# mfkiwl/msckf_stereo_c

Hardware: AMD Instinct MI355X
Metric: stereo frames/sec/node on EuRoC-shape input; ATE RMSE vs CPU ref (higher is better)
Workload: dtype f64

## Files before the change

### msckf_stereo_c_amd/csrc/hip/fe_kernels.hip

```cpp
#include <stdlib.h>
#include <mutex>
#include "fe_device.h"
#include "fe_mask.h"

__device__ __forceinline__ int reflect101(int i, int n) {
    if (n == 1) return 0;
    while (i < 0 || i >= n) { i = (i < 0) ? -i : 2 * (n - 1) - i; }
    return i;
}

#define P3_HALO 2
#define P3_OWN 12
#define P3_SEG_ROWS 8
struct Pyr3Job { const uint8_t *src; uint8_t *d1, *d2, *d3; int w0, h0; };

namespace {
typedef uint32_t __attribute__((aligned(1))) pd_u32u;
typedef uint16_t __attribute__((aligned(1))) pd_u16u;
typedef unsigned long long __attribute__((aligned(1))) pd_u64u;
typedef const __attribute__((address_space(1))) pd_u64u *pd_gld64;
typedef __attribute__((address_space(1))) pd_u32u *pd_gst32;
typedef __attribute__((address_space(1))) pd_u16u *pd_gst16;
typedef __attribute__((address_space(1))) uint8_t *pd_gst8;

// ... 209 lines not shown
    const int job = 4 * wi + (lane >> 4);
    const int seg = job / strips, strip = job - seg * strips;
    const int xs = DET_BORDER + DS_COLS * strip;
    const int ys = DET_BORDER + seg_rows * seg;
    const int y_end = min(ys + seg_rows, H - DET_BORDER);
    const bool job_on = xs < W - DET_BORDER && ys < y_end;
    if (!__any(job_on)) return;
    const int c0 = xs - 4 + 4 * r;
    const int cl = min(c0, W - 4);
    const uint8_t *img = S.curr0.lvl[0];
    typedef uint32_t __attribute__((aligned(1))) u32u;
    auto load = [&](int row) -> DetPix {
        const uint8_t *p = img + (size_t)min(max(row, 0), H - 1) * W + cl;
        DetPix v; v.lo = *(const u32u *)(p - 4); v.hi = *(const u32u *)p; return v;
    };
    int xin[4], cx[4];
    bool col_ok[4];
#pragma unroll
    for (int j = 0; j < 4; ++j) {
        const int x = c0 + 4 + j;
        cx[j] = x / cw; xin[j] = x - cx[j] * cw;
        col_ok[j] = job_on && r < DS_LANES && x < W - DET_BORDER;
    }
    const uint32_t *mrow = nullptr;
    int mpw = 0, msh = 0;
    if constexpr (MASKED) {
        mrow = masks[si].mask0; mpw = masks[si].pitch_w;
        if (mrow) mrow += min(c0 + 4, W - 1) >> 5;
        msh = (c0 + 4) & 31;
    }
    int Va[4] = {0, 0, 0, 0}, Vb[4] = {0, 0, 0, 0}, Vc[4] = {0, 0, 0, 0};
    int pr = ys - 4;
    DetPix e_mid = load(pr), e_dn = load(pr + 1), e_nx = load(pr + 2);
    uint32_t e_up = load(pr - 1).hi;
#pragma unroll 1
    for (int k = 0; k < 8; ++k) {
        const DetPix nx = load(pr + 3);
        int P[12];
        det_prod(e_up, e_mid, e_dn.hi, P);
        det_vadd(P, Va, Vb, Vc);
        e_up = e_mid.hi; e_mid = e_dn; e_dn = e_nx; e_nx = nx; ++pr;
    }
    uint32_t l_up = load(ys - 5).hi;
    DetPix l_mid = load(ys - 4), l_dn = load(ys - 3), l_nx = load(ys - 2);
    int cy = ys / ch, yin = ys - cy * ch;
    int bs[4] = {0, 0, 0, 0};
    unsigned long long bk[4] = {0ULL, 0ULL, 0ULL, 0ULL};
    const int n_rows = seg_rows;
#pragma unroll 1
    for (int k = 0; k < n_rows; ++k) {
        const int y = ys + k;
        const bool row_ok = y < y_end;
        const DetPix enx = load(pr + 3), lnx = load(y - 1);
        uint32_t nib = 15u;
        if constexpr (MASKED) { if (mrow) nib = (mrow[(size_t)min(y, H - 1) * mpw] >> msh) & 15u; }
        if (!MASKED || nib)
#pragma unroll
        for (int j = 0; j < 4; ++j) {
            if (!(col_ok[j] && row_ok)) continue;
            if (MASKED && !((nib >> j) & 1u)) continue;
            const int a = Va[j], b = Vb[j], d = Vc[j];
            const int X = (a + d) - max(det_floor, bs[j]);
            if (X <= 0) continue;
            const int df = a - d;
            if (abs(df) >= X || 2 * abs(b) >= X) continue;
            const double discd = (double)df * (double)df + 4.0 * ((double)b * (double)b);
            if (discd >= (double)X * (double)X) continue;
            const long long disc = (long long)df * df + 4LL * ((long long)b * b);
            const int score = (a + d) - (int)isqrt48((unsigned long long)disc, discd);
            bs[j] = score;
            bk[j] = det_key(gen, score, (unsigned int)(yin * cw + xin[j]));
        }
        {
            int Pe[12], Pl[12];
            det_prod(e_up, e_mid, e_dn.hi, Pe);
            det_prod(l_up, l_mid, l_dn.hi, Pl);
#pragma unroll
            for (int j = 0; j < 12; ++j) Pe[j] -= Pl[j];
            det_vadd(Pe, Va, Vb, Vc);
            e_up = e_mid.hi; e_mid = e_dn; e_dn = e_nx; e_nx = enx; ++pr;
            l_up = l_mid.hi; l_mid = l_dn; l_dn = l_nx; l_nx = lnx;
        }
        ++yin;
        const bool flush = job_on && row_ok && (yin == ch || y + 1 == y_end);
        if (cw < 4) {
            if (flush) {
#pragma unroll
                for (int j = 0; j < 4; ++j) {
                    if (bk[j]) atomicMax(&cell_keys[cy * det_cols + cx[j]], bk[j]);
                    bs[j] = 0; bk[j] = 0ULL;
                }
            }
        } else if (__any(flush)) {
            unsigned long long ka = 0ULL, kb = 0ULL;
#pragma unroll
            for (int j = 0; j < 4; ++j) {
                const unsigned long long v = flush ? bk[j] : 0ULL;
                if (cx[j] == cx[0]) ka = v > ka ? v : ka; else kb = v > kb ? v : kb;
            }
            const bool two = cx[3] != cx[0];
#pragma unroll 1
            for (int pass = 0; pass < 2; ++pass) {
                unsigned long long kk = pass ? kb : ka;
                const int id = flush ? (pass ? (two ? cx[3] : -1 - r) : cx[0]) : -1 - r;
                if (pass && !__any(flush && two)) break;
                {
                    const int o = det_dpp0<0x101>(id + 0x40000000) - 0x40000000; const unsigned long long v = det_dpp0_64<0x101>(kk);
                    if (o == id && v > kk) kk = v;
                }
                {
                    const int o = det_dpp0<0x102>(id + 0x40000000) - 0x40000000; const unsigned long long v = det_dpp0_64<0x102>(kk);
                    if (o == id && v > kk) kk = v;
                }
                {
                    const int o = det_dpp0<0x104>(id + 0x40000000) - 0x40000000; const unsigned long long v = det_dpp0_64<0x104>(kk);
                    if (o == id && v > kk) kk = v;
                }
                {
                    const int o = det_dpp0<0x108>(id + 0x40000000) - 0x40000000; const unsigned long long v = det_dpp0_64<0x108>(kk);
                    if (o == id && v > kk) kk = v;
                }
                const int left = det_dpp0<0x111>(id + 0x40000000) - 0x40000000;
                if (id >= 0 && left != id && kk) atomicMax(&cell_keys[cy * det_cols + id], kk);
            }
            if (flush) {
#pragma unroll
                for (int j = 0; j < 4; ++j) { bs[j] = 0; bk[j] = 0ULL; }
            }
        }
        if (yin == ch) { yin = 0; ++cy; }
    }
}

static void det_launch(const FeStreamDev *streams_dev, const FeMaskDev *masks_dev, int n_streams, int max_w, int max_h, unsigned int gen, hipStream_t st) {
    const int strips = (max_w - 2 * DET_BORDER + DS_COLS - 1) / DS_COLS, rows = max_h - 2 * DET_BORDER;
    if (strips <= 0 || rows <= 0) return;
    int seg_rows = 32;
    while (seg_rows < 128 && (long long)n_streams * strips * ((rows + seg_rows - 1) / seg_rows) / 4 > 32768) seg_rows *= 2;
    const int segs = (rows + seg_rows - 1) / seg_rows;
    const int waves = (strips * segs + 3) / 4;
    if (masks_dev) hipLaunchKernelGGL(k_detect_cells<true>, dim3(8 * ((n_streams + 7) / 8) * waves), dim3(64), 0, st, streams_dev, masks_dev, n_streams, strips, seg_rows, waves, gen);
    else hipLaunchKernelGGL(k_detect_cells<false>, dim3(8 * ((n_streams + 7) / 8) * waves), dim3(64), 0, st, streams_dev, masks_dev, n_streams, strips, seg_rows, waves, gen);
}
extern "C" void fe_launch_detect(const FeStreamDev *streams_dev, int n_streams, int max_w, int max_h, unsigned int gen, hipStream_t st) {
    det_launch(streams_dev, nullptr, n_streams, max_w, max_h, gen, st);
}
extern "C" void fe_launch_detect_masked(const FeStreamDev *streams_dev, const FeMaskDev *masks_dev, int n_streams, int max_w, int max_h, unsigned int gen, hipStream_t st) {
    if (!masks_dev) return;
    det_launch(streams_dev, masks_dev, n_streams, max_w, max_h, gen, st);
}

#include "fe_cam_models.h"

__device__ __forceinline__ void undistort_pt(const CamDev &cam, const double *R, float u, float v, float &xo, float &yo) {
    const double fx = cam.K[0], fy = cam.K[1], cx = cam.K[2], cy = cam.K[3];
    double x = ((double)u - cx) / fx, y = ((double)v - cy) / fy;
    if (cam.model == MSKF_MODEL_EQUIDISTANT) {
        const double *k = cam.D;
        double theta_d = sqrt(x * x + y * y);
        const double half_pi = 1.5707963267948966;
        theta_d = theta_d > half_pi ? half_pi : (theta_d < -half_pi ? -half_pi : theta_d);
        double scale = 0.0;
        if (theta_d > 1e-8) {
            double theta = theta_d;
            for (int j = 0; j < 10; ++j) {
                const double t2 = theta * theta, t4 = t2 * t2, t6 = t4 * t2, t8 = t6 * t2;
                const double k0t2 = k[0] * t2, k1t4 = k[1] * t4, k2t6 = k[2] * t6, k3t8 = k[3] * t8;
                const double fix = (theta * (1 + k0t2 + k1t4 + k2t6 + k3t8) - theta_d) /
                                   (1 + 3 * k0t2 + 5 * k1t4 + 7 * k2t6 + 9 * k3t8);
                theta = theta - fix;
                if (fabs(fix) < 1e-8) break;
            }
            scale = det_tan(theta) / theta_d;
        }
        x = x * scale; y = y * scale;
    } else {
        const double k1 = cam.D[0], k2 = cam.D[1], p1 = cam.D[2], p2 = cam.D[3];
        const double x0 = x, y0 = y;
        for (int j = 0; j < 5; ++j) {
            const double r2 = x * x + y * y;
            const double icdist = 1.0 / (1.0 + (k2 * r2 + k1) * r2);
            const double deltaX = 2.0 * p1 * x * y + p2 * (r2 + 2.0 * x * x);
            const double deltaY = p1 * (r2 + 2.0 * y * y) + 2.0 * p2 * x * y;
            x = (x0 - deltaX) * icdist;
            y = (y0 - deltaY) * icdist;
        }
    }
    if (R) {
        const double X = R[0] * x + R[1] * y + R[2];
        const double Y = R[3] * x + R[4] * y + R[5];
        const double Wd = R[6] * x + R[7] * y + R[8];
        x = X / Wd; y = Y / Wd;
    } else {
        x = x / 1.0; y = y / 1.0;
    }
    xo = (float)(x * 1.0 + 0.0);
    yo = (float)(y * 1.0 + 0.0);
}

__device__ __forceinline__ void distort_pt(const CamDev &cam, float xf, float yf, float &uo, float &vo) {
    const double fx = cam.K[0], fy = cam.K[1], cx = cam.K[2], cy = cam.K[3];
    const double x = (double)xf, y = (double)yf;
    double xd, yd;
    if (cam.model == MSKF_MODEL_EQUIDISTANT) {
        const double *k = cam.D;
        const double r = sqrt(x * x + y * y);
        const double theta = det_atan(r);
        const double t2 = theta * theta, t4 = t2 * t2, t6 = t4 * t2, t8 = t4 * t4;
        const double theta_d = theta * (1 + k[0] * t2 + k[1] * t4 + k[2] * t6 + k[3] * t8);
        const double scale = (r > 1e-8) ? theta_d / r : 1.0;
        xd = x * scale; yd = y * scale;
    } else {
        const double k1 = cam.D[0], k2 = cam.D[1], p1 = cam.D[2], p2 = cam.D[3];
        const double r2 = x * x + y * y, r4 = r2 * r2;
        const double a1 = 2.0 * x * y, a2 = r2 + 2.0 * x * x, a3 = r2 + 2.0 * y * y;
        const double cdist = 1.0 + k1 * r2 + k2 * r4;
        xd = x * cdist + p1 * a1 + p2 * a2;
        yd = y * cdist + p1 * a3 + p2 * a1;
    }
    uo = (float)(xd * fx + cx);
    vo = (float)(yd * fy + cy);
}

__device__ __forceinline__ bool undistort_pt_ext(const CamDev &cam, int model, const double *coef, const double *R, float u, float v, float &xo, float &yo) {
    if (model < FCM_RADTAN8) { undistort_pt(cam, R, u, v, xo, yo); return true; }
    return fcm_undistort_px(cam.K, model, coef, R, u, v, xo, yo);
}
__device__ __forceinline__ bool distort_pt_ext(const CamDev &cam, int model, const double *coef, float xf, float yf, float &uo, float &vo) {
    if (model < FCM_RADTAN8) { distort_pt(cam, xf, yf, uo, vo); return true; }
    return fcm_distort_px(cam.K, model, coef, xf, yf, uo, vo);
}

#include "fe_lk.h"

template <bool EXT>
__device__ __forceinline__ void track4_body(const FeStreamDev *streams, const FeCamExtDev *exts, int n_streams, int groups_per_stream,
                                            uint32_t (*s_T)[L4_TROWS * L4_DW + 2], uint32_t (*s_S)[L4_SROWS * L4_DW + 4]) {
    const int x = blockIdx.x & 7, qb = blockIdx.x >> 3;
    const int si = x + 8 * (qb / groups_per_stream), gi = qb - (qb / groups_per_stream) * groups_per_stream;
    if (si >= n_streams) return;
    const FeStreamDev &S = streams[si];
    const int n_pts = S.n_pts_dev ? *S.n_pts_dev : S.n_pts;
    const int lane = threadIdx.x & 63, g = lane >> 4, r = lane & 15;
    uint32_t *sT = s_T[g], *sS = s_S[g];
#pragma nounroll
    for (int gq = gi; 4 * gq < n_pts; gq += groups_per_stream) {
    const int pt = 4 * gq + g;
    const bool in_range = pt < n_pts;
    mskf_point2f pin = {0.f, 0.f};
    if (in_range) pin = S.in_pts[pt];
    unsigned int dbg_iters = 0, dbg_t = 0;
    float c0x = pin.x, c0y = pin.y;
    bool ok = in_range;
    float tx = 0.f, ty = 0.f, gx = 0.f, gy = 0.f;
    bool alive = false;
    int ph = 1;
    if (S.do_temporal) {
        const double *Hm = S.Hpred;
        const double px = (double)pin.x, py = (double)pin.y;
        const double X = Hm[0] * px + Hm[1] * py + Hm[2] * 1.0;
        const double Y = Hm[3] * px + Hm[4] * py + Hm[5] * 1.0;
        const double Z = Hm[6] * px + Hm[7] * py + Hm[8] * 1.0;
        tx = pin.x; ty = pin.y; gx = (float)(X / Z); gy = (float)(Y / Z);
        alive = in_range;
        ph = 0;
    }
    float c1x = 0.f, c1y = 0.f;
    int st1 = 0;
#pragma nounroll
    for (; ph < 2; ++ph) {
        if (ph == 1) {
            gx = 0.f; gy = 0.f;
            bool guessed = ok;
            if (ok) {
                float rx, ry;
                if (EXT) {
                    const FeCamExtDev &X = exts[si];
                    guessed = undistort_pt_ext(S.cam0, X.model[0], X.coef[0], S.R01, c0x, c0y, rx, ry);
                    if (guessed) guessed = distort_pt_ext(S.cam1, X.model[1], X.coef[1], rx, ry, gx, gy);
                    if (!guessed) { gx = 0.f; gy = 0.f; }
                } else {
                    undistort_pt(S.cam0, S.R01, c0x, c0y, rx, ry);
                    distort_pt(S.cam1, rx, ry, gx, gy);
                }
            }
            tx = c0x; ty = c0y; alive = guessed;
        }
        float nx = 0.f, ny = 0.f;
        int st = 0;
        if (__any(alive)) l4_track(ph ? S.curr0 : S.prev0, ph ? S.curr1 : S.curr0, alive, tx, ty, gx, gy, sT, sS, r, nx, ny, st, dbg_iters);
        if (ph == 0) {
            const int W = S.curr0.w[0], H = S.curr0.h[0];
            c0x = nx; c0y = ny;
            ok = alive && st != 0 && !(c0y < 0 || c0y > (float)(H - 1) || c0x < 0 || c0x > (float)(W - 1));
            dbg_t = dbg_iters; dbg_iters = 0;
        } else {
            c1x = alive ? nx : 0.f; c1y = alive ? ny : 0.f; st1 = alive ? st : 0;
        }
    }
    float u0x = 0.f, u0y = 0.f, u1x = 0.f, u1y = 0.f;
    int sst = st1;
    if (ok) {
        const int W1 = S.curr1.w[0], H1 = S.curr1.h[0];
        if (sst && (c1y < 0 || c1y > (float)(H1 - 1) || c1x < 0 || c1x > (float)(W1 - 1))) sst = 0;
        if (EXT) {
            const FeCamExtDev &X = exts[si];
            const bool in0 = undistort_pt_ext(S.cam0, X.model[0], X.coef[0], nullptr, c0x, c0y, u0x, u0y);
            const bool in1 = undistort_pt_ext(S.cam1, X.model[1], X.coef[1], nullptr, c1x, c1y, u1x, u1y);
            if (!in0 || !in1) sst = 0;
        } else {
            undistort_pt(S.cam0, nullptr, c0x, c0y, u0x, u0y);
            undistort_pt(S.cam1, nullptr, c1x, c1y, u1x, u1y);
        }
        if (sst) {
            const double *E = S.E;
            const double x0 = (double)u0x, y0 = (double)u0y, x1 = (double)u1x, y1 = (double)u1y;
            const double l0 = (E[0] * x0 + E[1] * y0) + E[2];
            const double l1 = (E[3] * x0 + E[4] * y0) + E[5];
            const double l2 = (E[6] * x0 + E[7] * y0) + E[8];
            const double err = fabs((x1 * l0 + y1 * l1) + l2) / sqrt(l0 * l0 + l1 * l1);
            if (err > S.epi_thresh) sst = 0;
        }
    }
    if (in_range && r == 0) {
        S.out0[pt] = mskf_point2f{c0x, c0y};
        S.out1[pt] = mskf_point2f{c1x, c1y};
        S.und0[pt] = mskf_point2f{u0x, u0y};
#ifdef LK_ITER_DBG
        ((unsigned int *)S.und1)[2 * pt] = dbg_t; ((unsigned int *)S.und1)[2 * pt + 1] = dbg_iters;
#else
        S.und1[pt] = mskf_point2f{u1x, u1y};
        (void)dbg_t;
#endif
        S.status[pt] = (uint8_t)(ok ? (1 | (sst ? 2 : 0)) : 0);
    }
    }
}
__global__ __launch_bounds__(64) void k_track4(const FeStreamDev *streams, int n_streams, int groups_per_stream) {
    __shared__ uint32_t s_T[4][L4_TROWS * L4_DW + 2];
    __shared__ uint32_t s_S[4][L4_SROWS * L4_DW + 4];
    track4_body<false>(streams, nullptr, n_streams, groups_per_stream, s_T, s_S);
}
__global__ __launch_bounds__(64) void k_track4_ext(const FeStreamDev *streams, const FeCamExtDev *exts, int n_streams, int groups_per_stream) {
    __shared__ uint32_t s_T[4][L4_TROWS * L4_DW + 2];
    __shared__ uint32_t s_S[4][L4_SROWS * L4_DW + 4];
    track4_body<true>(streams, exts, n_streams, groups_per_stream, s_T, s_S);
}

#include "fe_book.h"
__global__ __launch_bounds__(256) void k_fe_book(const FeBookDev *books, int which) {
    const FeBookDev &B = books[blockIdx.x];
    extern __shared__ int s_book[];
    FeBookScratch L;
    fe_book_scratch_init(L, s_book, B.cap, B.cand_cap, B.det_cap, B.n_codes, B.det_rows * B.det_cols);
    if (which == 0) fe_book1(B, L); else fe_book2(B, L);
}
extern "C" size_t fe_book_lds_budget(void) {
    static const size_t budget = []() -> size_t {
        const hipError_t e = hipFuncSetAttribute(reinterpret_cast<const void *>(k_fe_book), hipFuncAttributeMaxDynamicSharedMemorySize, 150 * 1024);
        if (e != hipSuccess) { (void)hipGetLastError(); return 64 * 1024; }
        return 150 * 1024;
    }();
    return budget;
}
extern "C" void fe_launch_book(const FeBookDev *books_dev, int n_streams, int which, size_t scratch_bytes, hipStream_t st) {
    (void)fe_book_lds_budget();
    hipLaunchKernelGGL(k_fe_book, dim3(n_streams), dim3(256), scratch_bytes, st, books_dev, which);
}

#include "fe_equalize.h"
namespace {
struct __attribute__((packed, aligned(1))) eq_u4 { uint32_t v[4]; };
__device__ __forceinline__ int eq_block_scan(int v, int *s, int tid) {
    s[tid] = v;
    __syncthreads();
    for (int off = 1; off < 256; off <<= 1) {
        const int t = tid >= off ? s[tid - off] : 0;
        __syncthreads();
        s[tid] += t;
        __syncthreads();
    }
    return s[tid];
}
__device__ __forceinline__ void eq_count16(int *hw, const uint32_t v[4], int lo, int hi) {
#pragma unroll
    for (int k = 0; k < 16; ++k)
        if (k >= lo && k < hi) atomicAdd(&hw[(v[k >> 2] >> (8 * (k & 3))) & 255u], 1);
}
}

__global__ __launch_bounds__(256) void k_eq_hist(const EqJob *jobs) {
    const EqJob j = jobs[blockIdx.y];
    const int unit = blockIdx.x, tid = threadIdx.x;
    const int n_units = j.mode == EQ_CLAHE ? j.tiles_x * j.tiles_y : j.n_strips;
    if (unit >= n_units) return;
    __shared__ int s_hist[4][256];
    __shared__ int s_scan[256];
#pragma unroll
    for (int k = 0; k < 4; ++k) s_hist[k][tid] = 0;
    __syncthreads();
    int r0, r1, c0, c1;
    if (j.mode == EQ_CLAHE) {
        const int ty = unit / j.tiles_x, tx = unit - ty * j.tiles_x;
        r0 = ty * j.th; r1 = r0 + j.th; c0 = tx * j.tw; c1 = c0 + j.tw;
    } else {
        r0 = unit * j.strip_rows; r1 = min(j.h, r0 + j.strip_rows); c0 = 0; c1 = j.w;
    }
    int *hw = s_hist[tid >> 6];
    const int w = j.w, h = j.h, cr = min(c1, w);
    if (cr > c0) {
        const uintptr_t img_b = (uintptr_t)j.src, img_e = img_b + (size_t)w * h;
        const int nch = (cr - c0 + 15) / 16 + 1;
        const int n_items = (r1 - r0) * nch;
        for (int idx = tid; idx < n_items; idx += 256) {
            const int rr = idx / nch, ch = idx - rr * nch;
            const uintptr_t a = img_b + (size_t)eq_src_row(r0 + rr, h) * w + c0, e = a + (size_t)(cr - c0);
            const uintptr_t q = (a & ~(uintptr_t)15) + 16 * (uintptr_t)ch;
            if (q >= e) continue;
            const int lo = a > q ? (int)(a - q) : 0, hi = e - q < 16 ? (int)(e - q) : 16;
            if (q >= img_b && q + 16 <= img_e) {
                const uint4 v = *reinterpret_cast<const uint4 *>(q);
                const uint32_t vv[4] = {v.x, v.y, v.z, v.w};
                eq_count16(hw, vv, lo, hi);
            } else {
                for (int k = lo; k < hi; ++k) atomicAdd(&hw[*reinterpret_cast<const uint8_t *>(q + k)], 1);
            }
        }
    }
    if (c1 > w) {
        const int cv0 = max(c0, w), nv = c1 - cv0, n_items = (r1 - r0) * nv;
        for (int idx = tid; idx < n_items; idx += 256) {
            const int rr = idx / nv, c = cv0 + idx - rr * nv;
            atomicAdd(&hw[j.src[(size_t)eq_src_row(r0 + rr, h) * w + eq_src_col(c, w)]], 1);
        }
    }
    __syncthreads();
    const int cnt = s_hist[0][tid] + s_hist[1][tid] + s_hist[2][tid] + s_hist[3][tid];
    if (j.mode != EQ_CLAHE) { j.part[256 * unit + tid] = cnt; return; }
    (void)eq_block_scan(eq_excess(cnt, j.clip), s_scan, tid);
    const int clipped = s_scan[255];
    __syncthreads();
    const int cum = eq_block_scan(eq_redistributed(cnt, tid, j.clip, clipped), s_scan, tid);
    j.lut[256 * (size_t)unit + tid] = (uint8_t)eq_clahe_entry(cum, eq_clahe_scale(j.tw * j.th));
}

__global__ __launch_bounds__(256) void k_eq_lut(const EqJob *jobs) {
    const EqJob j = jobs[blockIdx.x];
    if (j.mode != EQ_GLOBAL) return;
    const int tid = threadIdx.x;
    __shared__ int s_scan[256], s_cnt[256], s_i0;
    int cnt = 0;
    for (int s = 0; s < j.n_strips; ++s) cnt += j.part[256 * s + tid];
    s_cnt[tid] = cnt;
    if (tid == 0) s_i0 = 255;
    __syncthreads();
    if (cnt > 0) atomicMin(&s_i0, tid);
    const int cum = eq_block_scan(cnt, s_scan, tid);
    const int i0 = s_i0;
    j.lut[tid] = (uint8_t)eq_global_entry(tid, i0, s_cnt[i0], cum, j.w * j.h);
}

__global__ __launch_bounds__(256) void k_eq_apply(const EqJob *jobs, int splits) {
    const EqJob j = jobs[blockIdx.y];
    const int region = blockIdx.x / splits, split = blockIdx.x - region * splits, tid = threadIdx.x;
    if (region >= eq_regions(j.mode, j.tiles_x, j.tiles_y)) return;
    const bool clahe = j.mode == EQ_CLAHE;
    const int w = j.w, h = j.h;
    int x0 = 0, x1 = w, y0 = 0, y1 = h, t1x = 0, t2x = 0, t1y = 0, t2y = 0;
    float inv_tw = 0.f, inv_th = 0.f;
    if (clahe) {
        const int nrx = j.tiles_x + 1, ry = region / nrx, rx = region - ry * nrx;
        inv_tw = eq_inv(j.tw); inv_th = eq_inv(j.th);
        x0 = rx == 0 ? 0 : eq_axis_first(rx - 1, j.tw, inv_tw, w); x1 = rx == j.tiles_x ? w : eq_axis_first(rx, j.tw, inv_tw, w);
        y0 = ry == 0 ? 0 : eq_axis_first(ry - 1, j.th, inv_th, h); y1 = ry == j.tiles_y ? h : eq_axis_first(ry, j.th, inv_th, h);
        t1x = max(rx - 1, 0); t2x = min(rx, j.tiles_x - 1); t1y = max(ry - 1, 0); t2y = min(ry, j.tiles_y - 1);
    }
    const int rp = (y1 - y0 + splits - 1) / splits, ya = y0 + split * rp, yb = min(y1, ya + rp);
    if (ya >= yb || x0 >= x1) return;
    __shared__ uint32_t s_lut[256];
    if (clahe) {
        const uint8_t *r1 = j.lut + 256 * (size_t)(t1y * j.tiles_x), *r2 = j.lut + 256 * (size_t)(t2y * j.tiles_x);
        s_lut[tid] = (uint32_t)r1[256 * t1x + tid] | ((uint32_t)r1[256 * t2x + tid] << 8) | ((uint32_t)r2[256 * t1x + tid] << 16) | ((uint32_t)r2[256 * t2x + tid] << 24);
    } else s_lut[tid] = j.lut[tid];
    __syncthreads();
    const int nch = (x1 - x0 + 15) / 16 + 1, n_items = (yb - ya) * nch;
    for (int idx = tid; idx < n_items; idx += 256) {
        const int rr = idx / nch, ch = idx - rr * nch, y = ya + rr;
        const size_t row = (size_t)y * w, pb = row + x0, pe = row + x1;
        const size_t P = (pb & ~(size_t)15) + 16 * (size_t)ch;
        if (P >= pe) continue;
        const int lo = pb > P ? (int)(pb - P) : 0, hi = pe - P < 16 ? (int)(pe - P) : 16;
        const bool whole = lo == 0 && hi == 16;
        uint32_t in[4] = {0u, 0u, 0u, 0u}, out[4] = {0u, 0u, 0u, 0u};
        if (whole) { const eq_u4 v = *reinterpret_cast<const eq_u4 *>(j.src + P); in[0] = v.v[0]; in[1] = v.v[1]; in[2] = v.v[2]; in[3] = v.v[3]; }
        else {
#pragma unroll
            for (int k = 0; k < 16; ++k) if (k >= lo && k < hi) in[k >> 2] |= (uint32_t)j.src[P + k] << (8 * (k & 3));
        }
        EqAxis ay = {0, 0, 0.f, 0.f};
// ... 199 lines not shown
```

### msckf_stereo_c_amd/csrc/hip/fe_lk.h

```cpp
#pragma once
#include <hip/hip_runtime.h>
#include <stdint.h>
#include "fe_device.h"

#define LK_HALF 7
#define LK_WIN 15
#define LK_ITERS 30

template <int CTRL> __device__ __forceinline__ int dpp_add(int v) {
    return v + __builtin_amdgcn_update_dpp(0, v, CTRL, 0xf, 0xf, false);
}
__device__ __forceinline__ double lk_scaled_f64(long long b) {
    return __longlong_as_double(b + 0x41F8000000000000LL) - 6442450944.0;
}

typedef short l4_v2s __attribute__((ext_vector_type(2)));
#define L4_DW 6
#define L4_TROWS 18
#define L4_SROWS 20
#define L4_MAXOX 8
#define L4_MAXOY (L4_SROWS - 16)

typedef unsigned short l4_v2u __attribute__((ext_vector_type(2)));
template <int KA, int KC> __device__ __forceinline__ int l4_mad24_k(int x) {
    int d;
    asm("v_mad_i32_i24 %0, %1, %2, %3" : "=v"(d) : "n"(KA), "v"(x), "n"(KC));
    return d;
}
template <int KA> __device__ __forceinline__ int l4_mad24_kv(int x, int c) {
    int d;
    asm("v_mad_i32_i24 %0, %1, %2, %3" : "=v"(d) : "n"(KA), "v"(x), "v"(c));
    return d;
}
__device__ __forceinline__ int l4_mad24(int a, int b, int c) {
    int d;
    asm("v_mad_i32_i24 %0, %1, %2, %3" : "=v"(d) : "v"(a), "v"(b), "s"(c));
    return d;
}
__device__ __forceinline__ int l4_mad24_vvv(int a, int b, int c) {
    int d;
    asm("v_mad_i32_i24 %0, %1, %2, %3" : "=v"(d) : "v"(a), "v"(b), "v"(c));
    return d;
}
__device__ __forceinline__ int l4_dot2(int pair, int w, int acc) {
    return __builtin_amdgcn_sdot2(__builtin_bit_cast(l4_v2s, pair), __builtin_bit_cast(l4_v2s, w), acc, false);
}
__device__ __forceinline__ int l4_dot2k(int pair, int w, int k) {
    return __builtin_amdgcn_sdot2(__builtin_bit_cast(l4_v2s, pair), __builtin_bit_cast(l4_v2s, w), k, true);
}
__device__ __forceinline__ int l4_pack_shr9(int a, int b) {
    const l4_v2u v = __builtin_bit_cast(l4_v2u, __builtin_amdgcn_perm((uint32_t)b, (uint32_t)a, 0x06050201u));
    return __builtin_bit_cast(int, (l4_v2u)(v >> (unsigned short)1));
}
#define L4_SHL1 0x101
#define L4_SHR1 0x111
template <int CTRL> __device__ __forceinline__ int l4_dpp0(int v) {
    return __builtin_amdgcn_update_dpp(0, v, CTRL, 0xf, 0xf, true);
}
__device__ __forceinline__ long long l4_row_sum(int v) {
    v = dpp_add<0xB1>(v);
    v = dpp_add<0x4E>(v);
    long long s = (long long)v;
    {
        const int lo = __builtin_amdgcn_update_dpp(0, (int)s, 0x141, 0xf, 0xf, true), hi = __builtin_amdgcn_update_dpp(0, (int)(s >> 32), 0x141, 0xf, 0xf, true);
        s += (long long)(((unsigned long long)(unsigned int)hi << 32) | (unsigned int)lo);
    }
    {
        const int lo = __builtin_amdgcn_update_dpp(0, (int)s, 0x140, 0xf, 0xf, true), hi = __builtin_amdgcn_update_dpp(0, (int)(s >> 32), 0x140, 0xf, 0xf, true);
        s += (long long)(((unsigned long long)(unsigned int)hi << 32) | (unsigned int)lo);
    }
    return s;
}

struct __attribute__((packed, aligned(4))) l4_u4 { uint32_t v[4]; };
struct __attribute__((packed, aligned(4))) l4_u2 { uint32_t v[2]; };
template <int ROWS>
__device__ __forceinline__ void l4_stage(const uint8_t *img, int w, int h, int x0, int y0, uint32_t *dst, int r, bool on) {
    const bool fast = x0 >= 0 && y0 >= 0 && x0 + 4 * L4_DW <= w && y0 + ROWS <= h;
    if (fast) {
        if (on) {
            const uint8_t *p = img + l4_mad24_vvv(y0 + r, w, x0);
            const l4_u4 a = *(const l4_u4 *)p;
            const l4_u2 b = *(const l4_u2 *)(p + 16);
            uint32_t *d = dst + L4_DW * r;
            d[0] = a.v[0]; d[1] = a.v[1]; d[2] = a.v[2]; d[3] = a.v[3]; d[4] = b.v[0]; d[5] = b.v[1];
            if (r < ROWS - 16) {
                const uint8_t *p2 = img + l4_mad24_vvv(y0 + 16 + r, w, x0);
                const l4_u4 a2 = *(const l4_u4 *)p2;
                const l4_u2 b2 = *(const l4_u2 *)(p2 + 16);
                uint32_t *d2 = dst + L4_DW * (16 + r);
                d2[0] = a2.v[0]; d2[1] = a2.v[1]; d2[2] = a2.v[2]; d2[3] = a2.v[3]; d2[4] = b2.v[0]; d2[5] = b2.v[1];
            }
        }
        return;
    }
    constexpr int N = ROWS * L4_DW, PER = (N + 15) / 16;
    typedef uint32_t __attribute__((aligned(1))) l4_u32u;
    uint32_t v[PER];
#pragma unroll
    for (int i = 0; i < PER; ++i) {
        const int e = r + 16 * i;
        v[i] = 0;
        if (on && e < N) {
            const int row = (e * 43) >> 8, c = e - L4_DW * row;
            const uint8_t *rp = img + l4_mad24_vvv(min(max(y0 + row, 0), h - 1), w, 0);
            const int xb = x0 + 4 * c, xc = min(max(xb, 0), w - 4), sh = xb - xc;
            const uint32_t D = *(const l4_u32u *)(rp + xc);
            const uint32_t first = (D & 255u) * 0x01010101u, last = (D >> 24) * 0x01010101u;
            v[i] = sh < 0 ? first : sh >= 4 ? last : __builtin_amdgcn_alignbyte(last, D, (uint32_t)sh);
        }
    }
#pragma unroll
    for (int i = 0; i < PER; ++i) { const int e = r + 16 * i; if (on && e < N) dst[e] = v[i]; }
}

template <int K> __device__ __forceinline__ int l4_pair(const uint32_t *a) {
    constexpr int q = K >> 2, m = K & 3;
    if (m == 0) return (int)__builtin_amdgcn_perm(0u, a[q], 0x0c010c00u);
    if (m == 1) return (int)__builtin_amdgcn_perm(0u, a[q], 0x0c020c01u);
    if (m == 2) return (int)__builtin_amdgcn_perm(0u, a[q], 0x0c030c02u);
    return (int)__builtin_amdgcn_perm(a[q + 1], a[q], 0x0c040c03u);
}
template <int N, int K = 0> struct L4Pairs {
    static __device__ __forceinline__ void run(const uint32_t *a, int *pr) { pr[K] = l4_pair<K>(a); L4Pairs<N, K + 1>::run(a, pr); }
};
template <int N> struct L4Pairs<N, N> { static __device__ __forceinline__ void run(const uint32_t *, int *) {} };

__device__ __forceinline__ void l4_weights(float fa, float fb, int &wtop, int &wbot) {
    const int qa = __float2int_rn(fa * 16384.0f), qb = __float2int_rn(fb * 16384.0f);
    const int w00 = l4_mad24(16384 - qa, 16384 - qb, 8192) >> 14;
    const int w01 = l4_mad24(qa, 16384 - qb, 8192) >> 14;
    const int w10 = l4_mad24(16384 - qa, qb, 8192) >> 14;
    const int w11 = 16384 - w00 - w01 - w10;
    wtop = (w00 & 0xffff) | (w01 << 16);
    wbot = (w10 & 0xffff) | (w11 << 16);
}

__device__ __forceinline__ void l4_track(const PyrDev &A, const PyrDev &B, bool alive, float ax, float ay, float bx, float by,
                                         uint32_t *sT, uint32_t *sS, int r, float &out_x, float &out_y, int &out_status, unsigned int &dbg_iters) {
    int status = 1;
    float ncx = 0.f, ncy = 0.f;
    const bool winrow = r < LK_WIN;
    for (int l = MSKF_LEVELS - 1; l >= 0; --l) {
        const uint8_t *imA = A.lvl[l];
        const uint8_t *imB = B.lvl[l];
        const int aw = A.w[l], ah = A.h[l], bw = B.w[l], bh = B.h[l];
        const float sc = __int_as_float((127 - l) << 23);
        const float pwx = ax * sc - (float)LK_HALF, pwy = ay * sc - (float)LK_HALF;
        if (l == MSKF_LEVELS - 1) { ncx = bx * sc; ncy = by * sc; }
        else { ncx = ncx * 2.0f; ncy = ncy * 2.0f; }
        int ipx = (int)floorf(pwx), ipy = (int)floorf(pwy);
        bool lvl_on = alive && !(ipx < -LK_WIN || ipx >= aw || ipy < -LK_WIN || ipy >= ah);
        if (alive && !lvl_on && l == 0) status = 0;
        if (!lvl_on) { ipx = 0; ipy = 0; }
        int wtop, wbot;
        l4_weights(lvl_on ? pwx - (float)ipx : 0.f, lvl_on ? pwy - (float)ipy : 0.f, wtop, wbot);
        const int ax0 = (ipx - 1) & ~3, ay0 = ipy - 1, oxa = ipx - 1 - ax0;
        float wx = ncx - (float)LK_HALF, wy = ncy - (float)LK_HALF;
        int inx0 = (int)floorf(wx), iny0 = (int)floorf(wy);
        const bool in_b0 = !(inx0 < -LK_WIN || inx0 >= bw || iny0 < -LK_WIN || iny0 >= bh);
        if (!(lvl_on && in_b0)) { inx0 = 0; iny0 = 0; }
        int bx0 = (inx0 - 2) & ~3, by0 = iny0 - 2;
        __syncthreads();
        l4_stage<L4_TROWS>(imA, aw, ah, ax0, ay0, sT, r, true);
        l4_stage<L4_SROWS>(imB, bw, bh, bx0, by0, sS, r, true);
        __syncthreads();
        int V[17], E[17];
        {
            uint32_t d[6], a[5];
            int pr[17];
            const uint32_t *rp = sT + (r + 1) * L4_DW;
#pragma unroll
            for (int i = 0; i < 6; ++i) d[i] = rp[i];
#pragma unroll
            for (int i = 0; i < 5; ++i) a[i] = __builtin_amdgcn_alignbyte(d[i + 1], d[i], oxa);
            L4Pairs<17>::run(a, pr);
            int Bv[17];
#pragma unroll
            for (int c = 0; c < 17; ++c) { V[c] = l4_dot2k(pr[c], wtop, 256); Bv[c] = l4_dot2k(pr[c], wbot, 0); }
            const uint32_t *ep = sT + (r == 0 ? 0 : 17) * L4_DW;
#pragma unroll
            for (int i = 0; i < 6; ++i) d[i] = ep[i];
#pragma unroll
            for (int i = 0; i < 5; ++i) a[i] = __builtin_amdgcn_alignbyte(d[i + 1], d[i], oxa);
            L4Pairs<17>::run(a, pr);
            const int wsel = r == 0 ? wtop : wbot;
#pragma unroll
            for (int c = 0; c < 17; ++c) E[c] = l4_dot2(pr[c], wsel, r == 0 ? Bv[c] + 256 : V[c]) >> 9;
#pragma unroll
            for (int c = 0; c < 17; ++c) V[c] = (V[c] + l4_dpp0<L4_SHL1>(Bv[c])) >> 9;
            if (r == 15) {
#pragma unroll
                for (int c = 0; c < 17; ++c) V[c] = E[c];
            }
        }
        int Pp[8], Ixp[8], Iyp[8];
        int A11 = 0, A12 = 0, A22 = 0;
        {
            int f[17], e[17];
#pragma unroll
            for (int c = 0; c < 17; ++c) {
                const int up = __builtin_amdgcn_update_dpp(E[c], V[c], L4_SHR1, 0xf, 0xf, false);
                const int dn = l4_dpp0<L4_SHL1>(V[c]);
                f[c] = up + dn; e[c] = dn - up;
            }
            int gx[16], gy[16], pv[16];
#pragma unroll
            for (int i = 0; i < 15; ++i) {
                const int sx = l4_mad24_kv<10>(V[i + 2] - V[i], l4_mad24_k<3, 16>(f[i + 2] - f[i]));
                const int sy = l4_mad24_kv<10>(e[i + 1], l4_mad24_k<3, 16>(e[i] + e[i + 2]));
                gx[i] = sx >> 5;
                gy[i] = sy >> 5;
                pv[i] = V[i + 1];
            }
            gx[15] = 0; gy[15] = 0; pv[15] = 0;
#pragma unroll
            for (int m = 0; m < 8; ++m) {
                const int ix = (int)__builtin_amdgcn_perm((uint32_t)gx[2 * m + 1], (uint32_t)gx[2 * m], 0x05040100u);
                const int iy = (int)__builtin_amdgcn_perm((uint32_t)gy[2 * m + 1], (uint32_t)gy[2 * m], 0x05040100u);
                Ixp[m] = winrow ? ix : 0;
                Iyp[m] = winrow ? iy : 0;
                Pp[m] = (int)__builtin_amdgcn_perm((uint32_t)pv[2 * m + 1], (uint32_t)pv[2 * m], 0x05040100u);
                A11 = l4_dot2(Ixp[m], Ixp[m], A11); A12 = l4_dot2(Ixp[m], Iyp[m], A12); A22 = l4_dot2(Iyp[m], Iyp[m], A22);
            }
        }
        const long long A11s = l4_row_sum(A11), A12s = l4_row_sum(A12), A22s = l4_row_sum(A22);
        const double a11 = lk_scaled_f64(A11s), a12 = lk_scaled_f64(A12s), a22 = lk_scaled_f64(A22s);
        double D = a11 * a22 - a12 * a12;
        const double dd = a11 - a22;
        const double numer = a22 + a11 - sqrt(dd * dd + 4.0 * a12 * a12);
        bool run = lvl_on && !(numer < 0x1.70a3d70a3d70bp-5 || D < 1.1920928955078125e-07);
        if (lvl_on && !run && l == 0) status = 0;
        const bool solved = run;
        D = 1.0 / D;
        float pdx = 0.f, pdy = 0.f;
        for (int it = 0; it < LK_ITERS; ++it) {
            if (!__any(run)) break;
#ifdef LK_ITER_DBG
            if (run) dbg_iters += 1u << (8 * l);
#endif
            int inx = (int)floorf(wx), iny = (int)floorf(wy);
            if (run && (inx < -LK_WIN || inx >= bw || iny < -LK_WIN || iny >= bh)) {
                if (l == 0) status = 0;
                run = false;
            }
            int ox = inx - bx0, oy = iny - by0;
            const bool need = run && (ox < 0 || ox > L4_MAXOX || oy < 0 || oy > L4_MAXOY);
            if (__any(need)) {
                if (need) { bx0 = (inx - 2) & ~3; by0 = iny - 2; }
                __syncthreads();
                l4_stage<L4_SROWS>(imB, bw, bh, bx0, by0, sS, r, need);
                __syncthreads();
                ox = inx - bx0; oy = iny - by0;
            }
            if (!run) { ox = 0; oy = 0; }
            int wt, wb;
            l4_weights(wx - (float)inx, wy - (float)iny, wt, wb);
            uint32_t d[5], a[4];
            const uint32_t *rp = sS + l4_mad24_kv<L4_DW>(oy + r, ox >> 2);
#pragma unroll
            for (int i = 0; i < 5; ++i) d[i] = rp[i];
#pragma unroll
            for (int i = 0; i < 4; ++i) a[i] = __builtin_amdgcn_alignbyte(d[i + 1], d[i], ox & 3);
            int pr[15];
            L4Pairs<15>::run(a, pr);
            int sv[16];
#pragma unroll
            for (int k = 0; k < 15; ++k) {
                const int t = l4_dot2k(pr[k], wt, 256), b = l4_dot2k(pr[k], wb, 0);
                sv[k] = t + l4_dpp0<L4_SHL1>(b);
            }
            sv[15] = 0;
            int b1 = 0, b2 = 0;
#pragma unroll
            for (int m = 0; m < 8; ++m) {
                const l4_v2s sp = __builtin_bit_cast(l4_v2s, l4_pack_shr9(sv[2 * m], sv[2 * m + 1]));
                const int df = __builtin_bit_cast(int, (l4_v2s)(sp - __builtin_bit_cast(l4_v2s, Pp[m])));
                b1 = l4_dot2(df, Ixp[m], b1);
                b2 = l4_dot2(df, Iyp[m], b2);
            }
            const long long b1s = l4_row_sum(b1), b2s = l4_row_sum(b2);
            const double db1 = lk_scaled_f64(b1s), db2 = lk_scaled_f64(b2s);
            const float dx = (float)((a12 * db2 - a22 * db1) * D);
            const float dy = (float)((a12 * db1 - a11 * db2) * D);
            if (run) {
                wx += dx; wy += dy;
                if ((double)dx * (double)dx + (double)dy * (double)dy <= 1e-4) run = false;
                else if (it > 0 && fabsf(dx + pdx) < 0.01f && fabsf(dy + pdy) < 0.01f) {
                    wx -= dx * 0.5f; wy -= dy * 0.5f;
                    run = false;
                }
                pdx = dx; pdy = dy;
            }
        }
        if (solved) { ncx = wx + (float)LK_HALF; ncy = wy + (float)LK_HALF; }
    }
    out_x = ncx; out_y = ncy; out_status = status;
}
```

Measured before the change: 104,800.

## Fuse LK bilinear sampling via dot2c DPP asm and cache cam0 undistorted ray

Adds an inline-asm helper that does the bilinear vertical blend with v_dot2c_i32_i16_dpp row_shl, merging the bottom-row dot product and the DPP shift-add into one instruction. The helper is used in both the template build and the per-iteration LK sampling. The edge-row and template-row loads are reordered so the extra Bv array goes away, and a perm selector replaces the winrow selects. It also stores cam0's undistorted ray in shared memory during the stereo guess so the later undistortion reuses it instead of recomputing the iterative undistort. The inline asm relies on a manual s_nop hazard pad and exact DPP semantics, which is a correctness risk.

```diff
diff --git a/msckf_stereo_c_amd/csrc/hip/fe_kernels.hip b/msckf_stereo_c_amd/csrc/hip/fe_kernels.hip
--- a/msckf_stereo_c_amd/csrc/hip/fe_kernels.hip
+++ b/msckf_stereo_c_amd/csrc/hip/fe_kernels.hip
@@ -385,7 +385,7 @@
 
 #include "fe_cam_models.h"
 
-__device__ __forceinline__ void undistort_pt(const CamDev &cam, const double *R, float u, float v, float &xo, float &yo) {
+__device__ __forceinline__ void undistort_ray(const CamDev &cam, float u, float v, double &xr, double &yr) {
     const double fx = cam.K[0], fy = cam.K[1], cx = cam.K[2], cy = cam.K[3];
     double x = ((double)u - cx) / fx, y = ((double)v - cy) / fy;
     if (cam.model == MSKF_MODEL_EQUIDISTANT) {
@@ -419,6 +419,9 @@
             y = (y0 - deltaY) * icdist;
         }
     }
+    xr = x; yr = y;
+}
+__device__ __forceinline__ void undistort_rot(const double *R, double x, double y, float &xo, float &yo) {
     if (R) {
         const double X = R[0] * x + R[1] * y + R[2];
         const double Y = R[3] * x + R[4] * y + R[5];
@@ -429,6 +432,11 @@
     }
     xo = (float)(x * 1.0 + 0.0);
     yo = (float)(y * 1.0 + 0.0);
+}
+__device__ __forceinline__ void undistort_pt(const CamDev &cam, const double *R, float u, float v, float &xo, float &yo) {
+    double x, y;
+    undistort_ray(cam, u, v, x, y);
+    undistort_rot(R, x, y, xo, yo);
 }
 
 __device__ __forceinline__ void distort_pt(const CamDev &cam, float xf, float yf, float &uo, float &vo) {
@@ -468,7 +476,7 @@
 
 template <bool EXT>
 __device__ __forceinline__ void track4_body(const FeStreamDev *streams, const FeCamExtDev *exts, int n_streams, int groups_per_stream,
-                                            uint32_t (*s_T)[L4_TROWS * L4_DW + 2], uint32_t (*s_S)[L4_SROWS * L4_DW + 4]) {
+                                            uint32_t (*s_T)[L4_TROWS * L4_DW + 2], uint32_t (*s_S)[L4_SROWS * L4_DW + 4], double (*s_U)[2]) {
     const int x = blockIdx.x & 7, qb = blockIdx.x >> 3;
     const int si = x + 8 * (qb / groups_per_stream), gi = qb - (qb / groups_per_stream) * groups_per_stream;
     if (si >= n_streams) return;
@@ -513,7 +521,10 @@
                     if (guessed) guessed = distort_pt_ext(S.cam1, X.model[1], X.coef[1], rx, ry, gx, gy);
                     if (!guessed) { gx = 0.f; gy = 0.f; }
                 } else {
-                    undistort_pt(S.cam0, S.R01, c0x, c0y, rx, ry);
+                    double xr, yr;
+                    undistort_ray(S.cam0, c0x, c0y, xr, yr);
+                    s_U[g][0] = xr; s_U[g][1] = yr;
+                    undistort_rot(S.R01, xr, yr, rx, ry);
                     distort_pt(S.cam1, rx, ry, gx, gy);
                 }
             }
@@ -542,7 +553,7 @@
             const bool in1 = undistort_pt_ext(S.cam1, X.model[1], X.coef[1], nullptr, c1x, c1y, u1x, u1y);
             if (!in0 || !in1) sst = 0;
         } else {
-            undistort_pt(S.cam0, nullptr, c0x, c0y, u0x, u0y);
+            undistort_rot(nullptr, s_U[g][0], s_U[g][1], u0x, u0y);
             undistort_pt(S.cam1, nullptr, c1x, c1y, u1x, u1y);
         }
         if (sst) {
@@ -572,12 +583,13 @@
 __global__ __launch_bounds__(64) void k_track4(const FeStreamDev *streams, int n_streams, int groups_per_stream) {
     __shared__ uint32_t s_T[4][L4_TROWS * L4_DW + 2];
     __shared__ uint32_t s_S[4][L4_SROWS * L4_DW + 4];
-    track4_body<false>(streams, nullptr, n_streams, groups_per_stream, s_T, s_S);
+    __shared__ double s_U[4][2];
+    track4_body<false>(streams, nullptr, n_streams, groups_per_stream, s_T, s_S, s_U);
 }
 __global__ __launch_bounds__(64) void k_track4_ext(const FeStreamDev *streams, const FeCamExtDev *exts, int n_streams, int groups_per_stream) {
     __shared__ uint32_t s_T[4][L4_TROWS * L4_DW + 2];
     __shared__ uint32_t s_S[4][L4_SROWS * L4_DW + 4];
-    track4_body<true>(streams, exts, n_streams, groups_per_stream, s_T, s_S);
+    track4_body<true>(streams, exts, n_streams, groups_per_stream, s_T, s_S, nullptr);
 }
 
 #include "fe_book.h"
diff --git a/msckf_stereo_c_amd/csrc/hip/fe_lk.h b/msckf_stereo_c_amd/csrc/hip/fe_lk.h
--- a/msckf_stereo_c_amd/csrc/hip/fe_lk.h
+++ b/msckf_stereo_c_amd/csrc/hip/fe_lk.h
@@ -56,6 +56,23 @@
 #define L4_SHR1 0x111
 template <int CTRL> __device__ __forceinline__ int l4_dpp0(int v) {
     return __builtin_amdgcn_update_dpp(0, v, CTRL, 0xf, 0xf, true);
+}
+__device__ __forceinline__ void l4_sample5(const int *p, int wt, int wb, int *s) {
+    int s0, s1, s2, s3, s4;
+    asm("v_dot2_i32_i16 %0, %5, %10, %12\n\t"
+        "v_dot2_i32_i16 %1, %6, %10, %12\n\t"
+        "v_dot2_i32_i16 %2, %7, %10, %12\n\t"
+        "v_dot2_i32_i16 %3, %8, %10, %12\n\t"
+        "v_dot2_i32_i16 %4, %9, %10, %12\n\t"
+        "v_dot2c_i32_i16_dpp %0, %5, %11 row_shl:1 row_mask:0xf bank_mask:0xf bound_ctrl:1\n\t"
+        "v_dot2c_i32_i16_dpp %1, %6, %11 row_shl:1 row_mask:0xf bank_mask:0xf bound_ctrl:1\n\t"
+        "v_dot2c_i32_i16_dpp %2, %7, %11 row_shl:1 row_mask:0xf bank_mask:0xf bound_ctrl:1\n\t"
+        "v_dot2c_i32_i16_dpp %3, %8, %11 row_shl:1 row_mask:0xf bank_mask:0xf bound_ctrl:1\n\t"
+        "v_dot2c_i32_i16_dpp %4, %9, %11 row_shl:1 row_mask:0xf bank_mask:0xf bound_ctrl:1\n\t"
+        "s_nop 3"
+        : "=&v"(s0), "=&v"(s1), "=&v"(s2), "=&v"(s3), "=&v"(s4)
+        : "v"(p[0]), "v"(p[1]), "v"(p[2]), "v"(p[3]), "v"(p[4]), "v"(wt), "v"(wb), "s"(256));
+    s[0] = s0; s[1] = s1; s[2] = s2; s[3] = s3; s[4] = s4;
 }
 __device__ __forceinline__ long long l4_row_sum(int v) {
     v = dpp_add<0xB1>(v);
@@ -169,26 +186,29 @@
         {
             uint32_t d[6], a[5];
             int pr[17];
-            const uint32_t *rp = sT + (r + 1) * L4_DW;
-#pragma unroll
-            for (int i = 0; i < 6; ++i) d[i] = rp[i];
+            const uint32_t *ep = sT + (r == 0 ? 0 : 17) * L4_DW;
+#pragma unroll
+            for (int i = 0; i < 6; ++i) d[i] = ep[i];
 #pragma unroll
             for (int i = 0; i < 5; ++i) a[i] = __builtin_amdgcn_alignbyte(d[i + 1], d[i], oxa);
             L4Pairs<17>::run(a, pr);
-            int Bv[17];
-#pragma unroll
-            for (int c = 0; c < 17; ++c) { V[c] = l4_dot2k(pr[c], wtop, 256); Bv[c] = l4_dot2k(pr[c], wbot, 0); }
-            const uint32_t *ep = sT + (r == 0 ? 0 : 17) * L4_DW;
-#pragma unroll
-            for (int i = 0; i < 6; ++i) d[i] = ep[i];
+            const int wsel = r == 0 ? wtop : wbot, wother = r == 0 ? wbot : wtop;
+#pragma unroll
+            for (int c = 0; c < 17; ++c) E[c] = l4_dot2k(pr[c], wsel, 256);
+            const uint32_t *rp = sT + (r + 1) * L4_DW;
+#pragma unroll
+            for (int i = 0; i < 6; ++i) d[i] = rp[i];
 #pragma unroll
             for (int i = 0; i < 5; ++i) a[i] = __builtin_amdgcn_alignbyte(d[i + 1], d[i], oxa);
             L4Pairs<17>::run(a, pr);
-            const int wsel = r == 0 ? wtop : wbot;
-#pragma unroll
-            for (int c = 0; c < 17; ++c) E[c] = l4_dot2(pr[c], wsel, r == 0 ? Bv[c] + 256 : V[c]) >> 9;
-#pragma unroll
-            for (int c = 0; c < 17; ++c) V[c] = (V[c] + l4_dpp0<L4_SHL1>(Bv[c])) >> 9;
+#pragma unroll
+            for (int c = 0; c < 17; ++c) E[c] = l4_dot2(pr[c], wother, E[c]) >> 9;
+#pragma unroll
+            for (int c = 0; c < 15; c += 5) l4_sample5(pr + c, wtop, wbot, V + c);
+#pragma unroll
+            for (int c = 15; c < 17; ++c) V[c] = l4_dot2k(pr[c], wtop, 256) + l4_dpp0<L4_SHL1>(l4_dot2k(pr[c], wbot, 0));
+#pragma unroll
+            for (int c = 0; c < 17; ++c) V[c] = V[c] >> 9;
             if (r == 15) {
 #pragma unroll
                 for (int c = 0; c < 17; ++c) V[c] = E[c];
@@ -214,12 +234,11 @@
                 pv[i] = V[i + 1];
             }
             gx[15] = 0; gy[15] = 0; pv[15] = 0;
+            const uint32_t gsel = winrow ? 0x05040100u : 0x0c0c0c0cu;
 #pragma unroll
             for (int m = 0; m < 8; ++m) {
-                const int ix = (int)__builtin_amdgcn_perm((uint32_t)gx[2 * m + 1], (uint32_t)gx[2 * m], 0x05040100u);
-                const int iy = (int)__builtin_amdgcn_perm((uint32_t)gy[2 * m + 1], (uint32_t)gy[2 * m], 0x05040100u);
-                Ixp[m] = winrow ? ix : 0;
-                Iyp[m] = winrow ? iy : 0;
+                Ixp[m] = (int)__builtin_amdgcn_perm((uint32_t)gx[2 * m + 1], (uint32_t)gx[2 * m], gsel);
+                Iyp[m] = (int)__builtin_amdgcn_perm((uint32_t)gy[2 * m + 1], (uint32_t)gy[2 * m], gsel);
                 Pp[m] = (int)__builtin_amdgcn_perm((uint32_t)pv[2 * m + 1], (uint32_t)pv[2 * m], 0x05040100u);
                 A11 = l4_dot2(Ixp[m], Ixp[m], A11); A12 = l4_dot2(Ixp[m], Iyp[m], A12); A22 = l4_dot2(Iyp[m], Iyp[m], A22);
             }
@@ -266,10 +285,7 @@
             L4Pairs<15>::run(a, pr);
             int sv[16];
 #pragma unroll
-            for (int k = 0; k < 15; ++k) {
-                const int t = l4_dot2k(pr[k], wt, 256), b = l4_dot2k(pr[k], wb, 0);
-                sv[k] = t + l4_dpp0<L4_SHL1>(b);
-            }
+            for (int k = 0; k < 15; k += 5) l4_sample5(pr + k, wt, wb, sv + k);
             sv[15] = 0;
             int b1 = 0, b2 = 0;
 #pragma unroll
```

After: 108,200 (median of 6 runs). 3.2% higher.
